# Mariachiar/Spatiotemporal-Deepfake-Detection-for-Live-Video-Calls

Measured on AMD Instinct MI355X. Metric: clips/sec (32x3x224x224), higher is better.
Workload: dtype bf16

## Files before the change

### spatiotemporal-deepfake-detection-for-live-video-calls_amd/csrc/af_conv111.hip

```cpp
#include "af_common.h"
#include <stdlib.h>

namespace af {

struct C111Args {
    const char* in;
    const char* in2;
    const char* w;
    const char* w2;
    const float* scale;
    const float* shift;
    const char* res;
    char* out;
    int Cin, Cin2, Cout, out_ld, relu;
    int ncol;
    int T, HW, chunks;
    long long M;
    int tiles;
};

template <int NL, int NS, int D, int A = 0, int B = 0>
__device__ __forceinline__ void wait_counted(int nl, int ns) {
    if constexpr (A <= D - 1 && B <= D) {
        if (nl == A && ns == B) { wait_vmcnt<A * NL + B * NS>(); return; }
        if constexpr (B < D) wait_counted<NL, NS, D, A, B + 1>(nl, ns);
        else wait_counted<NL, NS, D, A + 1, 0>(nl, ns);
    } else {
        wait_vmcnt<0>();
    }
}

template <int DT, int KS1, int KS2, bool TPOOL, bool RES, int WC, int BM = 128, int NSLOT = 2>
__global__ __launch_bounds__(512, 1) void conv111_kernel(const C111Args a) {
    typedef Elem<DT> E;
    constexpr int EPC = E::EPC, ES = 16 / EPC;
    static_assert(EPC == 8, "16-bit storage types only");
    static_assert(WC == 64 || (WC == 32 && !TPOOL), "wave columns of 64 or 32 channels; the pooled tile order assumes 64");
    static_assert((BM == 128 || (BM == 64 && !TPOOL)) && NSLOT >= 2 && NSLOT <= 4, "tiles of 128 or 64 positions; the pooled row order assumes 128");
    constexpr int KS = KS1 + KS2, TN = WC / 16, D = NSLOT - 1;
    constexpr int NWN = 256 / WC, NWM = 8 / NWN, WPOS = BM / NWM, MT = WPOS / 16;
    constexpr int SLAB = BM * 128, STAGE = KS * SLAB;
    constexpr int PROW = WC + 4;
    constexpr int LPR = WC / 8, RPI = 64 / LPR, ITS = 16 / RPI;
    constexpr int NR = MT * ITS;
    constexpr int NPC = BM / 64;

    extern __shared__ uint4 smem[];
    const unsigned lds0 = (unsigned)(uintptr_t)(__attribute__((address_space(3))) char*)smem;
    const int tid = threadIdx.x, lane = tid & 63;
    const int wave = __builtin_amdgcn_readfirstlane(tid >> 6);
    const int frow = lane & 15, fg = lane >> 4;
    const int wn = wave % NWN, wm = wave / NWN;
    float* patch = reinterpret_cast<float*>(reinterpret_cast<char*>(smem) + NSLOT * STAGE) + wave * (16 * PROW);
    int col = blockIdx.x % a.ncol, first = blockIdx.x / a.ncol;
    const int stride = gridDim.x / a.ncol;
    if (gridDim.x % (8 * a.ncol) == 0) {
        const int xcd = blockIdx.x & 7, y = blockIdx.x >> 3;
        col = y % a.ncol;
        first = xcd + 8 * (y / a.ncol);
    }

    auto row_pixel = [&](int r) { return (r >> 6) * 32 + ((r >> 4) & 1) * 16 + (r & 15); };
    auto row_off = [&](int r) -> long long { return TPOOL ? (long long)((r >> 5) & 1) * a.HW + row_pixel(r) : r; };

    uint4 wreg[TN][2 * KS];
#pragma unroll
    for (int i = 0; i < TN; ++i) {
        const long long ch = col * 256 + wn * WC + i * 16 + frow;
#pragma unroll
        for (int k = 0; k < 2 * KS1; ++k)
            wreg[i][k] = *reinterpret_cast<const uint4*>(a.w + (ch * a.Cin + k * 32 + fg * 8) * ES);
#pragma unroll
        for (int k = 0; k < 2 * KS2; ++k)
            wreg[i][2 * KS1 + k] = *reinterpret_cast<const uint4*>(a.w2 + (ch * a.Cin2 + k * 32 + fg * 8) * ES);
    }

    constexpr bool REGEPI = WC == 32;
    const int rr = REGEPI ? frow : lane / LPR, cc = REGEPI ? (fg & 1) * 16 + (fg >> 1) * 8 : (lane % LPR) * 8;
    const int ch0 = col * 256 + wn * WC + cc;
    f32x4 sc[2], sf[2];
#pragma unroll
    for (int e = 0; e < 2; ++e) {
        const int chp = REGEPI ? col * 256 + wn * WC + e * 16 + fg * 4 : ch0 + 4 * e;
        sc[e] = *reinterpret_cast<const f32x4*>(a.scale + chp);
        sf[e] = *reinterpret_cast<const f32x4*>(a.shift + chp);
    }

    const int drow = lane >> 3, chunk = (lane & 7) ^ drow;
    const int xrow = wave * 8 + drow;
    const unsigned xoff = (unsigned)(row_off(xrow) * a.Cin * ES + chunk * 16);
    const unsigned x2off = KS2 ? (unsigned)(row_off(xrow) * a.Cin2 * ES + chunk * 16) : 0u;
    const int half_off = (int)(row_off(64) * a.Cin * ES), half2_off = (int)(row_off(64) * a.Cin2 * ES);
    auto tile_origin = [&](int tile, int& live) -> long long {
        if (TPOOL) {
            const int c = tile % a.chunks, nt = tile / a.chunks;
            live = a.HW - c * 64;
            return (long long)nt * 2 * a.HW + c * 64;
        }
        const long long o = (long long)tile * BM;
        live = (int)(a.M - o < BM ? a.M - o : BM);
        return o;
    };
    auto row_live = [&](int r, int live) { return TPOOL ? row_pixel(r) < live : r < live; };

    auto issue_tile = [&](int tile, int slot) {
        int live;
        const long long o = tile_origin(tile, live);
        const i32x4 d1 = make_desc(a.in + o * a.Cin * ES);
        const unsigned base = lds0 + slot * STAGE + wave * (8 * 128);
#pragma unroll
        for (int s = 0; s < KS1; ++s)
#pragma unroll
            for (int i = 0; i < NPC; ++i)
                blds16(row_live(xrow + 64 * i, live) ? xoff : kOutOfRange, d1, s * 128 + i * half_off, base + s * SLAB + i * (64 * 128));
        if (KS2) {
            const i32x4 d2 = make_desc(a.in2 + o * a.Cin2 * ES);
#pragma unroll
            for (int s = 0; s < KS2; ++s)
#pragma unroll
                for (int i = 0; i < NPC; ++i)
                    blds16(row_live(xrow + 64 * i, live) ? x2off : kOutOfRange, d2, s * 128 + i * half2_off, base + (KS1 + s) * SLAB + i * (64 * 128));
        }
    };
    const int row0 = wm * WPOS + rr;
    const unsigned res_lane = (unsigned)((row_off(row0) * a.Cout + ch0) * ES);
    const unsigned out_lane = (unsigned)(((long long)(TPOOL ? row_pixel(row0) : row0) * a.out_ld + ch0) * ES);
    auto k_row = [&](int k) { return (k / ITS) * 16 + (k % ITS) * RPI; };
    auto res_soff = [&](int k) { return (int)((row_off(k_row(k)) * a.Cout) * ES); };
    auto out_soff = [&](int k) { return (int)(((long long)(TPOOL ? row_pixel(k_row(k)) : k_row(k)) * a.out_ld) * ES); };
    auto load_residual = [&](int tile, u32x4 (&r)[NR]) {
        int live;
        const long long o = tile_origin(tile, live);
        const i32x4 rd = make_desc(a.res + o * a.Cout * ES);
#pragma unroll
        for (int k = 0; k < NR; ++k)
            r[k] = bload16_nt_uncounted(row_live(row0 + k_row(k), live) ? res_lane : kOutOfRange, rd, res_soff(k));
    };

    const int my_tiles = first < a.tiles ? (a.tiles - first + stride - 1) / stride : 0;
    u32x4 rs[NSLOT][NR];
#pragma unroll
    for (int u = 0; u < NSLOT; ++u)
#pragma unroll
        for (int k = 0; k < NR; ++k) rs[u][k] = u32x4{0u, 0u, 0u, 0u};
#pragma unroll
    for (int j = 0; j < D; ++j)
        if (j < my_tiles) {
            issue_tile(first + j * stride, j);
            if (RES) load_residual(first + j * stride, rs[j]);
        }
    __builtin_amdgcn_sched_barrier(0);
    constexpr int NL = KS * NPC + (RES ? NR : 0), NS = TPOOL ? NR / 2 : NR;
    static_assert((D - 1) * NL + D * NS <= 63, "vmcnt range");

    for (int q0 = 0; q0 < my_tiles; q0 += NSLOT) {
#pragma unroll
    for (int u = 0; u < NSLOT; ++u) {
        const int q = q0 + u;
        if (q >= my_tiles) break;
        const int tile = first + q * stride, slot = u;
        u32x4 (&rcur)[NR] = rs[u];
        if (D == 1) wait_vmcnt<0>();
        else {
            const int nl = my_tiles - 1 - q < D - 1 ? my_tiles - 1 - q : D - 1, ns = q < D ? q : D;
            wait_counted<NL, NS, D>(nl, ns);
        }
        __builtin_amdgcn_s_barrier();
        if (RES) {
#pragma unroll
            for (int k = 0; k < NR; ++k) asm volatile("" : "+v"(rcur[k]));
        }
        if (q + D < my_tiles) {
            issue_tile(tile + D * stride, (u + D) % NSLOT);
            if (RES) load_residual(tile + D * stride, rs[(u + D) % NSLOT]);
        }
        __builtin_amdgcn_sched_barrier(0);

        int live;
        const long long o = tile_origin(tile, live);
        const long long opos = TPOOL ? (o - o % a.HW) / 2 + o % a.HW : o;
        char* obase = a.out + opos * a.out_ld * ES;
        const uint4* xs = smem + slot * (STAGE / 16) + (wm * WPOS + frow) * 8;

#pragma unroll
        for (int h = 0; h < MT / 2; ++h) {
            f32x4 acc[TN][2];
#pragma unroll
            for (int i = 0; i < TN; ++i) { acc[i][0] = f32x4{0.f, 0.f, 0.f, 0.f}; acc[i][1] = f32x4{0.f, 0.f, 0.f, 0.f}; }
#pragma unroll
            for (int k = 0; k < 2 * KS; ++k) {
                const int c = ((k & 1) * 4 + fg) ^ (frow & 7);
                uint4 bf[2];
#pragma unroll
                for (int jl = 0; jl < 2; ++jl) bf[jl] = xs[(k >> 1) * (SLAB / 16) + (TPOOL ? h + 2 * jl : 2 * h + jl) * 16 * 8 + c];
#pragma unroll
                for (int i = 0; i < TN; ++i)
#pragma unroll
                    for (int jl = 0; jl < 2; ++jl) Mma<DT>::run(wreg[i][k], bf[jl], acc[i][jl]);
            }

            if constexpr (REGEPI) {
                const float lo = a.relu ? 0.f : -__builtin_inff();
#pragma unroll
                for (int jl = 0; jl < 2; ++jl) {
                    const int j = 2 * h + jl, row = wm * WPOS + j * 16 + rr;
                    f32x4 v0 = acc[0][jl] * sc[0] + sf[0], v1 = acc[1][jl] * sc[1] + sf[1];
                    if (RES) {
                        const u32x4 x = rcur[j];
                        const u32x2 s0 = __builtin_amdgcn_permlane16_swap(x[0], x[2], false, false);
                        const u32x2 s1 = __builtin_amdgcn_permlane16_swap(x[1], x[3], false, false);
                        const u32x2 ra = u32x2{s0[0], s1[0]}, rb = u32x2{s0[1], s1[1]};
                        v0 += Vec4<DT>::load(&ra); v1 += Vec4<DT>::load(&rb);
                    }
                    v0[0] = max_nan(v0[0], lo); v0[1] = max_nan(v0[1], lo); v0[2] = max_nan(v0[2], lo); v0[3] = max_nan(v0[3], lo);
                    v1[0] = max_nan(v1[0], lo); v1[1] = max_nan(v1[1], lo); v1[2] = max_nan(v1[2], lo); v1[3] = max_nan(v1[3], lo);
                    u32x2 p0, p1;
                    Vec4<DT>::store(&p0, v0); Vec4<DT>::store(&p1, v1);
                    const u32x4 o = swap_pair16(p0, p1);
                    if (row_live(row, live))
                        __builtin_nontemporal_store(o, reinterpret_cast<u32x4*>(obase + out_soff(j) + out_lane));
                }
                continue;
            }
            float keep[ITS][8];
#pragma unroll
            for (int jl = 0; jl < 2; ++jl) {
                const int j = TPOOL ? h + 2 * jl : 2 * h + jl;
#pragma unroll
                for (int i = 0; i < TN; ++i)
                    *reinterpret_cast<f32x4*>(patch + frow * PROW + i * 16 + fg * 4) = acc[i][jl];
                __builtin_amdgcn_wave_barrier();
#pragma unroll
                for (int it = 0; it < ITS; ++it) {
                    const int prow = it * RPI + rr, row = wm * WPOS + j * 16 + prow;
                    float v[8];
#pragma unroll
                    for (int e = 0; e < 8; e += 4) {
                        const f32x4 t = *reinterpret_cast<const f32x4*>(patch + prow * PROW + cc + e);
                        const f32x4 r = t * sc[e >> 2] + sf[e >> 2];
                        v[e] = r[0]; v[e + 1] = r[1]; v[e + 2] = r[2]; v[e + 3] = r[3];
                    }
                    if (RES) {
                        const uint4 rraw = __builtin_bit_cast(uint4, rcur[j * ITS + it]);
                        const typename E::type* re = reinterpret_cast<const typename E::type*>(&rraw);
#pragma unroll
                        for (int e = 0; e < 8; ++e) v[e] += E::to_f32(re[e]);
                    }
                    if (a.relu) {
#pragma unroll
                        for (int e = 0; e < 8; ++e) v[e] = relu_f(v[e]);
                    }
                    if (TPOOL && jl == 0) {
#pragma unroll
                        for (int e = 0; e < 8; ++e) keep[it][e] = v[e];
                        continue;
                    }
                    if (TPOOL) {
#pragma unroll
                        for (int e = 0; e < 8; ++e) v[e] = max_nan(keep[it][e], v[e]);
                    }
                    uint4 ov;
                    typename E::type* oe = reinterpret_cast<typename E::type*>(&ov);
#pragma unroll
                    for (int e = 0; e < 8; ++e) oe[e] = E::from_f32(v[e]);
                    if (row_live(row, live))
                        __builtin_nontemporal_store(__builtin_bit_cast(u32x4, ov), reinterpret_cast<u32x4*>(obase + out_soff(j * ITS + it) + out_lane));
                }
                __builtin_amdgcn_wave_barrier();
            }
        }
    }
    }
}

template <int DT, int KS1, int KS2, bool TPOOL, bool RES, int WC = 64, int BM = 128, int NSLOT = 2>
static int launch111(const C111Args& a, int blocks, hipStream_t stream) {
    const int lds = NSLOT * (KS1 + KS2) * BM * 128 + 8 * 16 * (WC + 4) * 4;
    AF_SET_MAX_LDS((&conv111_kernel<DT, KS1, KS2, TPOOL, RES, WC, BM, NSLOT>), lds, "conv111");
    hipLaunchKernelGGL((conv111_kernel<DT, KS1, KS2, TPOOL, RES, WC, BM, NSLOT>), dim3(blocks), dim3(512), lds, stream, a);
    AF_CHECK_LAUNCH("conv111_kernel");
    return AF_OK;
}

static int conv111_bm(const af_conv_desc* d) { return d->cin >= 128 ? 64 : 128; }

static long long conv111_tiles(const af_conv_desc* d, const af_conv_desc* d2, int out_ld) {
    if (d->dtype == AF_F32) return 0;
    if (d->kt != 1 || d->kh != 1 || d->kw != 1 || d->st != 1 || d->sh != 1 || d->sw != 1 || d->pt || d->ph || d->pw) return 0;
    if (d->cout % 256 != 0 || (d->tpool != 0 && d->tpool != 1)) return 0;
    if (d2) {
        if (d->cin != 64 || d2->cin != 64 || d->tpool) return 0;
        if (d2->st != 1 || d2->sh != 1 || d2->sw != 1 || d2->t != d->t || d2->h != d->h || d2->w != d->w) return 0;
    } else if (d->cin != 64 && d->cin != 128 && d->cin != 256) return 0;
    if (d->tpool && (d->cin != 64 || d->t % 2 != 0)) return 0;
    const long long hw = (long long)d->h * d->w;
    if ((hw + 128) * 128 * 2 * 2 >= (1LL << 31)) return 0;
    const int bm = conv111_bm(d);
    const long long tiles = d->tpool ? (long long)d->n * (d->t / 2) * ((hw + 63) / 64) : ((long long)d->n * d->t * hw + bm - 1) / bm;
    if (tiles >= (1LL << 30)) return 0;
    if (tiles * bm / 128 * (d->cout / 256) < 4LL * device_cus()) return 0;
    return tiles;
}

bool conv111_applies(const af_conv_desc* d, const af_conv_desc* d2, const void* residual, int out_ld) {
    if (d2 && residual) return false;
    return conv111_tiles(d, d2, out_ld) != 0;
}

int conv111_run(const af_conv_desc* d, const void* in, const void* w_packed, const af_conv_desc* d2, const void* in2,
                const void* w2_packed, const float* scale, const float* shift, const void* residual, void* out, int out_ld,
                hipStream_t stream) {
    C111Args a;
    a.in = (const char*)in; a.in2 = (const char*)in2; a.w = (const char*)w_packed; a.w2 = (const char*)w2_packed;
    a.scale = scale; a.shift = shift; a.res = (const char*)residual; a.out = (char*)out;
    a.Cin = d->cin; a.Cin2 = d2 ? d2->cin : 0; a.Cout = d->cout; a.out_ld = out_ld; a.relu = d->relu;
    a.ncol = d->cout / 256;
    a.T = d->t; a.HW = d->h * d->w; a.chunks = (a.HW + 63) / 64;
    a.M = (long long)d->n * d->t * a.HW;
    a.tiles = (int)conv111_tiles(d, d2, out_ld);
    int streams = device_cus() / a.ncol;
    if (streams > a.tiles) streams = a.tiles;
    const int blocks = streams * a.ncol;
    const bool bf = d->dtype == AF_BF16;
#define AF_C111(K1, K2, TP, RS) (bf ? launch111<AF_BF16, K1, K2, TP, RS>(a, blocks, stream) : launch111<AF_F16, K1, K2, TP, RS>(a, blocks, stream))
    if (d2) return AF_C111(1, 1, false, false);
    if (d->tpool) return residual ? AF_C111(1, 0, true, true) : AF_C111(1, 0, true, false);
    if (d->cin == 64) return residual ? AF_C111(1, 0, false, true) : AF_C111(1, 0, false, false);
    if (d->cin == 256) {
        const char* ewc = getenv("AF_C111_WC64");
        if (!(ewc && atoi(ewc) == 0))
            return residual ? (bf ? launch111<AF_BF16, 4, 0, false, true, 64, 64, 2>(a, blocks, stream) : launch111<AF_F16, 4, 0, false, true, 64, 64, 2>(a, blocks, stream))
                            : (bf ? launch111<AF_BF16, 4, 0, false, false, 64, 64, 2>(a, blocks, stream) : launch111<AF_F16, 4, 0, false, false, 64, 64, 2>(a, blocks, stream));
        return residual ? (bf ? launch111<AF_BF16, 4, 0, false, true, 32, 64, 4>(a, blocks, stream) : launch111<AF_F16, 4, 0, false, true, 32, 64, 4>(a, blocks, stream))
                        : (bf ? launch111<AF_BF16, 4, 0, false, false, 32, 64, 4>(a, blocks, stream) : launch111<AF_F16, 4, 0, false, false, 32, 64, 4>(a, blocks, stream));
    }
    return residual ? (bf ? launch111<AF_BF16, 2, 0, false, true, 64, 64, 4>(a, blocks, stream) : launch111<AF_F16, 2, 0, false, true, 64, 64, 4>(a, blocks, stream))
                    : (bf ? launch111<AF_BF16, 2, 0, false, false, 64, 64, 4>(a, blocks, stream) : launch111<AF_F16, 2, 0, false, false, 64, 64, 4>(a, blocks, stream));
#undef AF_C111
}

}
```

Before: 3422.

## Fuse strided-downsample shortcut 1x1 conv into conv111 via gathered second input

Adds a gathered second-input mode so a stride-2 1x1 downsample projection (cin 256) can be fused with the cin-128 expansion 1x1 conv in one kernel. Row addresses for the second input are computed with magic-number division. It also extends conv111 to cin=512, raises the minimum work threshold for cin 128/256, caches the getenv lookup, and changes the direct-epilogue stores from nontemporal to regular. The aim is to remove a separate downsample conv launch and its output round trip, plus route more layers to the tuned kernel. The risks are the extra per-tile index arithmetic and strided second-input loads.

```diff
diff --git a/spatiotemporal-deepfake-detection-for-live-video-calls_amd/csrc/af_conv111.hip b/spatiotemporal-deepfake-detection-for-live-video-calls_amd/csrc/af_conv111.hip
--- a/spatiotemporal-deepfake-detection-for-live-video-calls_amd/csrc/af_conv111.hip
+++ b/spatiotemporal-deepfake-detection-for-live-video-calls_amd/csrc/af_conv111.hip
@@ -17,7 +17,19 @@
     int T, HW, chunks;
     long long M;
     int tiles;
+    int W, H, F2, RH2, SW2;
+    unsigned dw_m, dw_l, dh_m, dh_l;
 };
+
+__device__ __forceinline__ unsigned fdiv32(unsigned x, unsigned m, unsigned l) {
+    const unsigned t = __umulhi(m, x);
+    return l == 0 ? x : (t + ((x - t) >> 1)) >> (l - 1);
+}
+static void magic32(unsigned d, unsigned& m, unsigned& l) {
+    l = 0;
+    while ((1ull << l) < d) ++l;
+    m = (unsigned)(((1ull << 32) * ((1ull << l) - d)) / d + 1);
+}
 
 template <int NL, int NS, int D, int A = 0, int B = 0>
 __device__ __forceinline__ void wait_counted(int nl, int ns) {
@@ -30,13 +42,14 @@
     }
 }
 
-template <int DT, int KS1, int KS2, bool TPOOL, bool RES, int WC, int BM = 128, int NSLOT = 2>
+template <int DT, int KS1, int KS2, bool TPOOL, bool RES, int WC, int BM = 128, int NSLOT = 2, bool G2 = false>
 __global__ __launch_bounds__(512, 1) void conv111_kernel(const C111Args a) {
     typedef Elem<DT> E;
     constexpr int EPC = E::EPC, ES = 16 / EPC;
     static_assert(EPC == 8, "16-bit storage types only");
     static_assert(WC == 64 || (WC == 32 && !TPOOL), "wave columns of 64 or 32 channels; the pooled tile order assumes 64");
     static_assert((BM == 128 || (BM == 64 && !TPOOL)) && NSLOT >= 2 && NSLOT <= 4, "tiles of 128 or 64 positions; the pooled row order assumes 128");
+    static_assert(!G2 || (KS2 > 0 && BM == 64 && !TPOOL), "a gathered second input: one DMA piece per wave and K slab, no pooling");
     constexpr int KS = KS1 + KS2, TN = WC / 16, D = NSLOT - 1;
     constexpr int NWN = 256 / WC, NWM = 8 / NWN, WPOS = BM / NWM, MT = WPOS / 16;
     constexpr int SLAB = BM * 128, STAGE = KS * SLAB;
@@ -114,12 +127,23 @@
             for (int i = 0; i < NPC; ++i)
                 blds16(row_live(xrow + 64 * i, live) ? xoff : kOutOfRange, d1, s * 128 + i * half_off, base + s * SLAB + i * (64 * 128));
         if (KS2) {
-            const i32x4 d2 = make_desc(a.in2 + o * a.Cin2 * ES);
+            unsigned off2 = x2off;
+            long long o2 = o;
+            if (G2) {
+                auto row2 = [&](unsigned m) {
+                    const unsigned q = fdiv32(m, a.dw_m, a.dw_l), nt = fdiv32(q, a.dh_m, a.dh_l);
+                    return nt * (unsigned)a.F2 + (q - nt * a.H) * (unsigned)a.RH2 + (m - q * a.W) * (unsigned)a.SW2;
+                };
+                const unsigned r0 = row2((unsigned)o);
+                o2 = r0;
+                off2 = (row2((unsigned)o + xrow) - r0) * (unsigned)(a.Cin2 * ES) + chunk * 16;
+            }
+            const i32x4 d2 = make_desc(a.in2 + o2 * a.Cin2 * ES);
 #pragma unroll
             for (int s = 0; s < KS2; ++s)
 #pragma unroll
                 for (int i = 0; i < NPC; ++i)
-                    blds16(row_live(xrow + 64 * i, live) ? x2off : kOutOfRange, d2, s * 128 + i * half2_off, base + (KS1 + s) * SLAB + i * (64 * 128));
+                    blds16(row_live(xrow + 64 * i, live) ? off2 : kOutOfRange, d2, s * 128 + i * half2_off, base + (KS1 + s) * SLAB + i * (64 * 128));
         }
     };
     const int row0 = wm * WPOS + rr;
@@ -218,7 +242,7 @@
                     Vec4<DT>::store(&p0, v0); Vec4<DT>::store(&p1, v1);
                     const u32x4 o = swap_pair16(p0, p1);
                     if (row_live(row, live))
-                        __builtin_nontemporal_store(o, reinterpret_cast<u32x4*>(obase + out_soff(j) + out_lane));
+                        *reinterpret_cast<u32x4*>(obase + out_soff(j) + out_lane) = o;
                 }
                 continue;
             }
@@ -273,32 +297,42 @@
     }
 }
 
-template <int DT, int KS1, int KS2, bool TPOOL, bool RES, int WC = 64, int BM = 128, int NSLOT = 2>
+template <int DT, int KS1, int KS2, bool TPOOL, bool RES, int WC = 64, int BM = 128, int NSLOT = 2, bool G2 = false>
 static int launch111(const C111Args& a, int blocks, hipStream_t stream) {
-    const int lds = NSLOT * (KS1 + KS2) * BM * 128 + 8 * 16 * (WC + 4) * 4;
-    AF_SET_MAX_LDS((&conv111_kernel<DT, KS1, KS2, TPOOL, RES, WC, BM, NSLOT>), lds, "conv111");
-    hipLaunchKernelGGL((conv111_kernel<DT, KS1, KS2, TPOOL, RES, WC, BM, NSLOT>), dim3(blocks), dim3(512), lds, stream, a);
+    const int lds = NSLOT * (KS1 + KS2) * BM * 128 + (WC == 32 ? 0 : 8 * 16 * (WC + 4) * 4);
+    static_assert(NSLOT * (KS1 + KS2) * BM * 128 + (WC == 32 ? 0 : 8 * 16 * (WC + 4) * 4) <= 160 * 1024, "LDS");
+    AF_SET_MAX_LDS((&conv111_kernel<DT, KS1, KS2, TPOOL, RES, WC, BM, NSLOT, G2>), lds, "conv111");
+    hipLaunchKernelGGL((conv111_kernel<DT, KS1, KS2, TPOOL, RES, WC, BM, NSLOT, G2>), dim3(blocks), dim3(512), lds, stream, a);
     AF_CHECK_LAUNCH("conv111_kernel");
     return AF_OK;
 }
 
 static int conv111_bm(const af_conv_desc* d) { return d->cin >= 128 ? 64 : 128; }
+
+static bool conv111_gathered(const af_conv_desc* d, const af_conv_desc* d2) {
+    return d2 && d->cin == 128 && d2->cin == 256 && d2->kt == 1 && d2->kh == 1 && d2->kw == 1 && !d2->pt && !d2->ph && !d2->pw &&
+           d2->st == 1 && d2->sh == 2 && d2->sw == 2 && d2->t == d->t && (d2->h - 1) / 2 + 1 == d->h && (d2->w - 1) / 2 + 1 == d->w;
+}
 
 static long long conv111_tiles(const af_conv_desc* d, const af_conv_desc* d2, int out_ld) {
     if (d->dtype == AF_F32) return 0;
     if (d->kt != 1 || d->kh != 1 || d->kw != 1 || d->st != 1 || d->sh != 1 || d->sw != 1 || d->pt || d->ph || d->pw) return 0;
     if (d->cout % 256 != 0 || (d->tpool != 0 && d->tpool != 1)) return 0;
     if (d2) {
-        if (d->cin != 64 || d2->cin != 64 || d->tpool) return 0;
-        if (d2->st != 1 || d2->sh != 1 || d2->sw != 1 || d2->t != d->t || d2->h != d->h || d2->w != d->w) return 0;
-    } else if (d->cin != 64 && d->cin != 128 && d->cin != 256) return 0;
+        if (d->tpool) return 0;
+        const bool same = d->cin == 64 && d2->cin == 64 && d2->st == 1 && d2->sh == 1 && d2->sw == 1 && d2->t == d->t &&
+                          d2->h == d->h && d2->w == d->w;
+        if (!same && !conv111_gathered(d, d2)) return 0;
+    } else if (d->cin != 64 && d->cin != 128 && d->cin != 256 && d->cin != 512) return 0;
     if (d->tpool && (d->cin != 64 || d->t % 2 != 0)) return 0;
     const long long hw = (long long)d->h * d->w;
     if ((hw + 128) * 128 * 2 * 2 >= (1LL << 31)) return 0;
     const int bm = conv111_bm(d);
     const long long tiles = d->tpool ? (long long)d->n * (d->t / 2) * ((hw + 63) / 64) : ((long long)d->n * d->t * hw + bm - 1) / bm;
     if (tiles >= (1LL << 30)) return 0;
-    if (tiles * bm / 128 * (d->cout / 256) < 4LL * device_cus()) return 0;
+    const long long units = tiles * (d->cout / 256);
+    const bool kept = !d2 && (d->cin == 128 || d->cin == 256);
+    if (units < (kept ? 8LL : 4LL) * device_cus()) return 0;
     return tiles;
 }
 
@@ -318,17 +352,30 @@
     a.T = d->t; a.HW = d->h * d->w; a.chunks = (a.HW + 63) / 64;
     a.M = (long long)d->n * d->t * a.HW;
     a.tiles = (int)conv111_tiles(d, d2, out_ld);
+    a.W = d->w; a.H = d->h; a.F2 = a.RH2 = a.SW2 = 0;
+    a.dw_m = a.dw_l = a.dh_m = a.dh_l = 0;
+    const bool gathered = conv111_gathered(d, d2);
+    if (gathered) {
+        a.F2 = d2->h * d2->w; a.RH2 = d2->sh * d2->w; a.SW2 = d2->sw;
+        magic32((unsigned)d->w, a.dw_m, a.dw_l);
+        magic32((unsigned)d->h, a.dh_m, a.dh_l);
+    }
     int streams = device_cus() / a.ncol;
     if (streams > a.tiles) streams = a.tiles;
     const int blocks = streams * a.ncol;
     const bool bf = d->dtype == AF_BF16;
 #define AF_C111(K1, K2, TP, RS) (bf ? launch111<AF_BF16, K1, K2, TP, RS>(a, blocks, stream) : launch111<AF_F16, K1, K2, TP, RS>(a, blocks, stream))
+    if (gathered) return bf ? launch111<AF_BF16, 2, 4, false, false, 32, 64, 3, true>(a, blocks, stream)
+                            : launch111<AF_F16, 2, 4, false, false, 32, 64, 3, true>(a, blocks, stream);
     if (d2) return AF_C111(1, 1, false, false);
     if (d->tpool) return residual ? AF_C111(1, 0, true, true) : AF_C111(1, 0, true, false);
     if (d->cin == 64) return residual ? AF_C111(1, 0, false, true) : AF_C111(1, 0, false, false);
+    if (d->cin == 512)
+        return residual ? (bf ? launch111<AF_BF16, 8, 0, false, true, 32, 64, 2>(a, blocks, stream) : launch111<AF_F16, 8, 0, false, true, 32, 64, 2>(a, blocks, stream))
+                        : (bf ? launch111<AF_BF16, 8, 0, false, false, 32, 64, 2>(a, blocks, stream) : launch111<AF_F16, 8, 0, false, false, 32, 64, 2>(a, blocks, stream));
     if (d->cin == 256) {
-        const char* ewc = getenv("AF_C111_WC64");
-        if (!(ewc && atoi(ewc) == 0))
+        static const bool wc64 = [] { const char* e = getenv("AF_C111_WC64"); return !(e && atoi(e) == 0); }();
+        if (wc64)
             return residual ? (bf ? launch111<AF_BF16, 4, 0, false, true, 64, 64, 2>(a, blocks, stream) : launch111<AF_F16, 4, 0, false, true, 64, 64, 2>(a, blocks, stream))
                             : (bf ? launch111<AF_BF16, 4, 0, false, false, 64, 64, 2>(a, blocks, stream) : launch111<AF_F16, 4, 0, false, false, 64, 64, 2>(a, blocks, stream));
         return residual ? (bf ? launch111<AF_BF16, 4, 0, false, true, 32, 64, 4>(a, blocks, stream) : launch111<AF_F16, 4, 0, false, true, 32, 64, 4>(a, blocks, stream))
```

Result: no change. 3449, median of 6 (+0.8%).
